# chalharu/rust-compression

Hardware: AMD Instinct MI355X
Metric: BZip2 level-9 encode MB/s (input bytes, HBM-resident in and out: the kernels' rate; value_end_to_end is host buffer to host buffer at the C ABI) (higher is better)
Workload: dtype u8/u32

## Files before the change

rust-compression_amd/csrc/k_huff.hip:

```cpp
#include "bzgpu.h"
#include <cstdlib>

namespace bzgpu {

constexpr u32 kHuffThreads = 512;

__device__ __forceinline__ u32 weight_add(u32 x, u32 y)
{
    const u32 dx = x & 0xFFu, dy = y & 0xFFu;
    return ((x & 0xFFFFFF00u) + (y & 0xFFFFFF00u)) | (1u + (dx > dy ? dx : dy));
}

__device__ void down_heap(u32 *buf, u32 nn, u32 len)
{
    const u32 tmp = buf[nn];
    u32 leaf = (nn << 1) + 1;
    while (leaf < len) {
        if (leaf + 1 < len && buf[buf[leaf]] > buf[buf[leaf + 1]]) leaf += 1;
        if (buf[tmp] < buf[buf[leaf]]) break;
        buf[nn] = buf[leaf];
        nn = leaf;
        leaf = (nn << 1) + 1;
    }
    buf[nn] = tmp;
// ... 966 lines not shown
                    nacc -= 32u;
                }
            }
        }
        if (nacc) atomicOr(&s_buf[widx], (u32)(acc >> 32));
    }
    __syncthreads();
    for (u32 q = tid * 4u; q < nwords; q += kEmitThreads * 4u) {
        const u32 w = base + q;
        if (w > wf && w + 3u < wl && w + 3u < kStreamWords) {
            *reinterpret_cast<uint4 *>(stream + w) = *reinterpret_cast<const uint4 *>(s_buf + q);
            continue;
        }
#pragma unroll
        for (u32 j = 0; j < 4; ++j) {
            const u32 ww = w + j;
            if (ww < wf || ww > wl || ww >= kStreamWords) continue;
            const u32 v = s_buf[q + j];
            if (ww != wf && ww != wl) stream[ww] = v;
            else if (v) atomicOr(&stream[ww], v);
        }
    }
}

constexpr u32 kSweepThreads = 256;
constexpr u32 kSweepTilesX = 11;
constexpr u32 kTabArena = 6 * (3 * kMaxAlpha + 4);

__device__ __forceinline__ u32 huff_group_num(u32 mtf_count)
{
    if (mtf_count < 200) return 2;
    if (mtf_count < 600) return 3;
    if (mtf_count < 1200) return 4;
    if (mtf_count < 2400) return 5;
    return 6;
}

__device__ __forceinline__ void lm_wave_sync()
{
    __builtin_amdgcn_fence(__ATOMIC_ACQ_REL, "workgroup");
    __builtin_amdgcn_wave_barrier();
}
__device__ void lm_code_lengths_wave(const u32 *rfreq, u32 n, u32 *scr, u32 scr_words, u32 row, u8 *out, u32 lane)
{
    const u32 lim = kLim;
    u32 *map = scr;
    u32 *sfreq = map + kMaxAlpha;
    u32 *c = sfreq + kMaxAlpha;
    u32 *misc = c + kMaxAlpha;
    u32 *max_elem = misc, *b = misc + 20, *cur = misc + 40;
    u32 *val = misc + 64 + kMaxAlpha;
    u32 *ty = val + lim * row;
    u32 *w = scr + scr_words - kMaxAlpha;
    for (u32 i = lane; i < n; i += 64u) {
        const u32 f = rfreq[i];
        w[i] = (f > 1u ? f : 1u) << 8;
    }
    lm_wave_sync();
    for (u32 i = lane; i < n; i += 64u) {
        const u32 f = w[i];
        u32 r = 0;
        for (u32 q = 0; q < n; ++q) {
            const u32 x = w[q];
            r += (x > f || (x == f && q < i)) ? 1u : 0u;
        }
        sfreq[r] = f;
        map[r] = i;
    }
    if (lane == 0) {
        for (u32 j = 0; j < lim; ++j) { max_elem[j] = 0; b[j] = 0; cur[j] = 0; }
        u32 excess = (1u << lim) - n;
        const u32 half = 1u << (lim - 1);
        max_elem[lim - 1] = n;
        for (u32 j = 0; j < lim; ++j) {
            if (excess >= half) {
                b[j] = 1;
                excess -= half;
            }
            excess <<= 1;
            if (lim >= 2 + j) max_elem[lim - 2 - j] = max_elem[lim - 1 - j] / 2 + n;
        }
        max_elem[0] = b[0];
        for (u32 j = 1; j < lim; ++j)
            if (max_elem[j] > 2 * max_elem[j - 1] + b[j]) max_elem[j] = 2 * max_elem[j - 1] + b[j];
    }
    lm_wave_sync();
    for (u32 j = 0; j < lim; ++j)
        for (u32 t = lane; t < max_elem[j]; t += 64u) { val[j * row + t] = 0; ty[j * row + t] = 0; }
    for (u32 i = lane; i < n; i += 64u) c[i] = lim;
    lm_wave_sync();
    for (u32 t = lane; t < n && t < max_elem[lim - 1]; t += 64u) {
        val[(lim - 1) * row + t] = sfreq[t];
        ty[(lim - 1) * row + t] = t;
    }
    if (lane == 0 && b[lim - 1] == 1) {
        c[0] -= 1;
        cur[lim - 1] += 1;
    }
    lm_wave_sync();
    const u32 last_leaf = sfreq[n - 1];
    for (u32 j = lim - 1; j > 0;) {
        const u32 next0 = cur[j], me = max_elem[j], cap = max_elem[j - 1];
        const u32 K = (me > next0 + 1u) ? (me - next0) / 2u : 0u;
        u32 *vj = val + j * row, *dv = val + (j - 1) * row, *dt = ty + (j - 1) * row;
        for (u32 k0 = 0; k0 < K; k0 += 64u) {
            const u32 k = k0 + lane;
            u32 pk = 0;
            if (k < K) pk = weight_add(vj[next0 + 2u * k], vj[next0 + 2u * k + 1u]);
            lm_wave_sync();
            if (k < K) vj[k] = pk;
        }
        lm_wave_sync();
        for (u32 k = lane; k < K; k += 64u) {
            const u32 pk = vj[k];
            if (pk > last_leaf) {
                u32 lo = 0, hi = n;
                while (lo < hi) {
                    const u32 mid = (lo + hi) >> 1;
                    if (sfreq[mid] >= pk) lo = mid + 1u;
                    else hi = mid;
                }
                const u32 pos = k + lo;
                if (pos < cap) {
                    dv[pos] = pk;
                    dt[pos] = n;
                }
            }
        }
        for (u32 i = lane; i < n; i += 64u) {
            const u32 sf = sfreq[i];
            u32 lo = 0, hi = K;
            while (lo < hi) {
                const u32 mid = (lo + hi) >> 1;
                if (vj[mid] > sf) lo = mid + 1u;
                else hi = mid;
            }
            const u32 pos = i + lo;
            if (pos < cap) {
                dv[pos] = sf;
                dt[pos] = i;
            }
        }
        lm_wave_sync();
        j -= 1;
        if (lane == 0) cur[j] = 0;
        lm_wave_sync();
        if (b[j] == 1) {
            u32 need = 1;
            for (u32 li = j; need > 0u && li < lim; ++li) {
                const u32 c0 = cur[li];
                u32 npk = 0;
                for (u32 t0 = 0; t0 < need; t0 += 64u) {
                    const u32 t = t0 + lane;
                    bool isp = false;
                    if (t < need) {
                        const u32 x = ty[li * row + c0 + t];
                        if (x == n) isp = true;
                        else c[x] -= 1;
                    }
                    npk += (u32)__popcll(__ballot(isp));
                }
                lm_wave_sync();
                if (lane == 0) cur[li] = c0 + need;
                need = 2u * npk;
                lm_wave_sync();
            }
        }
        lm_wave_sync();
    }
    for (u32 i = lane; i < n; i += 64u) out[map[i]] = (u8)c[i];
    lm_wave_sync();
}

template <u32 THREADS>
__device__ __forceinline__ void stage_symbols_n(u32 *s_sym, const u16 *__restrict__ mtf, u32 g0, u32 mtf_count)
{
    const u32 first = g0 * kGSize;
    const u32 avail = mtf_count - first;
    const u32 want = THREADS * kGSize;
    const u32 nsym = avail < want ? avail : want;
    const u32 ndw = (nsym + 1u) >> 1;
    const u32 *src = reinterpret_cast<const u32 *>(mtf + first);
    u32 v[kGSize / 2];
#pragma unroll
    for (u32 k = 0; k < kGSize / 2; ++k) {
        const u32 i = threadIdx.x + k * THREADS;
        v[k] = (i < ndw) ? src[i] : 0u;
    }
#pragma unroll
    for (u32 k = 0; k < kGSize / 2; ++k) {
        const u32 i = threadIdx.x + k * THREADS;
        if (i < ndw) s_sym[i] = v[k];
    }
}

constexpr u32 kTabPipeBlocks = 320;
template <u32 kTabThreads>
__global__ __launch_bounds__(kTabThreads) void k_huff_tables(HuffArgs a, u32 iter)
{
    __shared__ u8 s_len[6][kMaxAlpha + 6];
    __shared__ u32 s_rfreq[6][kMaxAlpha];
    __shared__ __attribute__((aligned(16))) u32 s_arena[kTabArena];
    __shared__ u32 s_need[6];
    __shared__ u32 s_lmcount;
    static_assert(kTabArena >= 6 * (3 * kMaxAlpha + 4) && (3 * kMaxAlpha + 4) % 2 == 0, "the heap work arrays fit the arena, 8-byte aligned");
    const u32 lb = blockIdx.x, tid = threadIdx.x, lane = threadIdx.x & 63u, wv = threadIdx.x >> 6;
    const BlockOut &bo = a.out[lb];
    const u32 mtf_count = bo.mtf_count;
    const u32 alpha = bo.in_use_count + 2;
    const u32 group_num = huff_group_num(mtf_count);
    const u32 *mtf_freq = a.mtf_freq + (size_t)lb * kMaxAlpha;
    u32 *rfreq = a.rfreq + (size_t)lb * 6 * kMaxAlpha;
    u8 *glen = a.glen + (size_t)lb * 6 * (kMaxAlpha + 6);
    const bool tab_lane = tid < group_num;
    const u32 tb = tid;
    if (tid == 0) s_lmcount = 0;
    if (iter == 0) {
        if (tid == 0) {
            u32 rem = mtf_count;
            int gs = 0;
            for (u32 k = 0; k < group_num; ++k) {
                const u32 n_part = group_num - k;
                const u32 t_freq = rem / n_part;
                int ge = gs - 1;
                u32 a_freq = 0;
                while (a_freq < t_freq && ge < (int)alpha - 1) {
                    ge += 1;
                    a_freq += mtf_freq[ge];
                }
                if (ge > gs && n_part != group_num && n_part != 1 && (((group_num - n_part) & 1u) == 1u)) {
                    a_freq -= mtf_freq[ge];
                    ge -= 1;
                }
                s_need[group_num - 1 - k] = (u32)gs | ((u32)(ge + 1) << 16);
                rem -= a_freq;
                gs = ge + 1;
            }
            a.hlm[lb] = 0;
        }
        for (u32 i = tid; i < 6 * kMaxAlpha; i += kTabThreads) rfreq[i] = 0;
        __syncthreads();
        for (u32 i = tid; i < group_num * alpha; i += kTabThreads) {
            const u32 t = i / alpha, sym = i - t * alpha, rg = s_need[t];
            s_len[t][sym] = (sym >= (rg & 0xFFFFu) && sym < (rg >> 16)) ? 0 : 15;
        }
        __syncthreads();
    } else {
        for (u32 i = tid; i < 6 * kMaxAlpha; i += kTabThreads) {
            (&s_rfreq[0][0])[i] = rfreq[i];
            rfreq[i] = 0;
        }
        __syncthreads();
        if constexpr (kTabThreads >= 384) {
            const bool on = wv < group_num;
            const u32 gq = on ? wv : 0u;
            const int lm = heap_code_lengths_pipe(s_rfreq[gq], alpha, s_arena + gq * (3 * kMaxAlpha + 4), s_len[gq], lane, on);
            if (on && lane == 0) s_need[wv] = (u32)lm;
        } else {
            if (tab_lane) s_need[tb] = (u32)heap_code_lengths_w(s_rfreq[tb], alpha, s_arena + tb * (3 * kMaxAlpha + 4), s_len[tb]);
        }
        __syncthreads();
        const u32 row = 2u * alpha + 4u;
        const u32 need = 5u * kMaxAlpha + 64u + 2u * kLim * row;
        const u32 slots = kTabArena / need;
        u32 my_rank = 0, any = 0;
        for (u32 t = 0; t < group_num; ++t) {
            if (t < tb) my_rank += s_need[t] ? 1u : 0u;
            any += s_need[t] ? 1u : 0u;
        }
        (void)my_rank;
        if (any) {
            if (slots) {
                if (wv == 0) {
                    for (u32 t = 0; t < group_num; ++t) {
                        if (s_need[t]) {
                            lm_code_lengths_wave(s_rfreq[t], alpha, s_arena, need, row, s_len[t], lane);
                            if (lane == 0) s_lmcount += 1;
                        }
                    }
                }
                __syncthreads();
            } else {
                for (u32 t = wv; t < group_num; t += kTabThreads / 64u) {
                    if (s_need[t]) {
                        lm_code_lengths_wave(s_rfreq[t], alpha, a.lm_scratch + ((size_t)lb * 6 + t) * kLmWords, kLmWords, kLmRow,
                                             s_len[t], lane);
                        if (lane == 0) atomicAdd(&s_lmcount, 1u);
                    }
                }
                __syncthreads();
            }
        }
    }
    for (u32 i = tid; i < 6 * (kMaxAlpha + 6); i += kTabThreads) glen[i] = (&s_len[0][0])[i];
    unsigned long long *pack = a.pack + (size_t)lb * kMaxAlpha;
    for (u32 i = tid; i < alpha; i += kTabThreads) {
        unsigned long long p = 0;
        for (u32 t = 0; t < group_num; ++t) p |= (unsigned long long)s_len[t][i] << (10 * t);
        pack[i] = p;
    }
    if (tid == 0 && s_lmcount) a.hlm[lb] += s_lmcount;
}

__global__ __launch_bounds__(kSweepThreads) void k_huff_sweep(HuffArgs a, u32 iter)
{
    __shared__ unsigned long long s_pack[kMaxAlpha];
    __shared__ u32 s_pass[8];
    __shared__ u32 s_rfreq[6][kMaxAlpha];
    __shared__ u32 s_sym[kSweepThreads * kGSize / 2];
    const u32 lb = blockIdx.y, tid = threadIdx.x;
    const u32 mtf_count = a.out[lb].mtf_count;
    const u32 n_selectors = (mtf_count + kGSize - 1) / kGSize;
    if (blockIdx.x * kSweepThreads >= n_selectors) return;
    const u32 alpha = a.out[lb].in_use_count + 2;
    const u32 group_num = huff_group_num(mtf_count);
    const u16 *mtf = a.mtf + (size_t)lb * a.mtf_stride;
    u8 *selector = a.selector + (size_t)lb * kSelStride;
    const unsigned long long *pack = a.pack + (size_t)lb * kMaxAlpha;
    for (u32 i = tid; i < alpha; i += kSweepThreads) s_pack[i] = pack[i];
    for (u32 i = tid; i < 6 * kMaxAlpha; i += kSweepThreads) (&s_rfreq[0][0])[i] = 0;
    if (tid < 8) s_pass[tid] = 0;
    for (u32 g0 = blockIdx.x * kSweepThreads; g0 < n_selectors; g0 += kSweepTilesX * kSweepThreads) {
        __syncthreads();
        stage_symbols_n<kSweepThreads>(s_sym, mtf, g0, mtf_count);
        __syncthreads();
        const u32 g = g0 + tid;
        u32 bt_mine = 0xFFFFFFFFu, bc_mine = 0;
        if (g < n_selectors) {
            const u32 gs = g * kGSize;
            const u32 cnt = (gs + kGSize < mtf_count) ? kGSize : mtf_count - gs;
            const u32 *my = s_sym + tid * (kGSize / 2);
            unsigned long long cost = 0, c8 = 0;
            u32 big = 0;
            if (cnt == kGSize) {
#pragma unroll 5
                for (u32 k = 0; k < kGSize / 2; ++k) {
                    const u32 dw = my[k];
                    const u32 s0 = dw & 0xFFFFu, s1 = dw >> 16;
                    cost += s_pack[s0];
                    cost += s_pack[s1];
                    if (s0 < 8u) c8 += 1ull << (8u * s0);
                    else ++big;
                    if (s1 < 8u) c8 += 1ull << (8u * s1);
                    else ++big;
                }
            } else {
                for (u32 i = 0; i < cnt; ++i) {
                    const u32 sy = (my[i >> 1] >> ((i & 1u) * 16u)) & 0xFFFFu;
                    cost += s_pack[sy];
                    if (sy < 8u) c8 += 1ull << (8u * sy);
                    else ++big;
                }
            }
            u32 bt = 0, bc = (u32)(cost & 1023u);
            for (u32 t = 1; t < group_num; ++t) {
                const u32 ct = (u32)((cost >> (10 * t)) & 1023u);
                if (ct < bc) {
                    bc = ct;
                    bt = t;
                }
            }
            selector[g] = (u8)bt;
            bt_mine = bt;
            bc_mine = bc;
            if (big) {
                for (u32 i = 0; i < cnt; ++i) {
                    const u32 sy = (my[i >> 1] >> ((i & 1u) * 16u)) & 0xFFFFu;
                    if (sy >= 8u) atomicAdd(&s_rfreq[bt][sy], 1u);
                }
            }
#pragma unroll
            for (u32 q = 0; q < 8; ++q) {
                const u32 c = (u32)(c8 >> (8u * q)) & 0xFFu;
                if (c) atomicAdd(&s_rfreq[bt][q], c);
            }
        }
        if (a.pass_stats) {
            const u32 wtot = wave_sum(bc_mine);
            u32 mine = 0;
#pragma unroll
            for (u32 t = 0; t < 6; ++t) {
                const u32 c = (u32)__popcll(__ballot(bt_mine == t));
                mine = (tid & 63u) == t + 1u ? c : mine;
            }
            if ((tid & 63u) == 0u) mine = wtot;
            if ((tid & 63u) < 7u && mine) atomicAdd(&s_pass[tid & 63u], mine);
        }
    }
    __syncthreads();
    u32 *rfreq = a.rfreq + (size_t)lb * 6 * kMaxAlpha;
    for (u32 i = tid; i < group_num * kMaxAlpha; i += kSweepThreads) {
        const u32 c = (&s_rfreq[0][0])[i];
        if (c) atomicAdd(&rfreq[i], c);
    }
    if (a.pass_stats && tid < 7 && s_pass[tid]) atomicAdd(&a.pass_stats[((size_t)lb * 4 + iter) * 8 + tid], s_pass[tid]);
}

__global__ __launch_bounds__(kSweepThreads) void k_huff_gbits(HuffArgs a)
{
    __shared__ u8 s_len[6][kMaxAlpha + 6];
    __shared__ u32 s_sym[kSweepThreads * kGSize / 2];
    const u32 lb = blockIdx.y, tid = threadIdx.x;
    const u32 mtf_count = a.out[lb].mtf_count;
    const u32 n_selectors = (mtf_count + kGSize - 1) / kGSize;
    if (blockIdx.x * kSweepThreads >= n_selectors) return;
    const u16 *mtf = a.mtf + (size_t)lb * a.mtf_stride;
    const u8 *selector = a.selector + (size_t)lb * kSelStride;
    const u8 *glen = a.glen + (size_t)lb * 6 * (kMaxAlpha + 6);
    u32 *gbo = a.group_bitoff + (size_t)lb * kGboStride;
    for (u32 i = tid; i < 6 * (kMaxAlpha + 6); i += kSweepThreads) (&s_len[0][0])[i] = glen[i];
    for (u32 g0 = blockIdx.x * kSweepThreads; g0 < n_selectors; g0 += kSweepTilesX * kSweepThreads) {
        __syncthreads();
        stage_symbols_n<kSweepThreads>(s_sym, mtf, g0, mtf_count);
        __syncthreads();
        const u32 g = g0 + tid;
        if (g < n_selectors) {
            const u32 gs = g * kGSize;
            const u32 cnt = (gs + kGSize < mtf_count) ? kGSize : mtf_count - gs;
            const u32 *my = s_sym + tid * (kGSize / 2);
            const u8 *l = s_len[selector[g]];
            u32 bits = 0;
            if (cnt == kGSize) {
#pragma unroll 5
                for (u32 k = 0; k < kGSize / 2; ++k) {
                    const u32 d = my[k];
                    bits += (u32)l[d & 0xFFFFu] + (u32)l[d >> 16];
                }
            } else {
                for (u32 i = 0; i < cnt; ++i) bits += l[(my[i >> 1] >> ((i & 1u) * 16u)) & 0xFFFFu];
            }
            gbo[g] = bits;
        }
    }
}

__global__ __launch_bounds__(kHuffThreads) void k_huff_header(HuffArgs a)
{
    __shared__ u8 s_len[6][kMaxAlpha + 6];
    __shared__ u32 s_scan[kHuffThreads / 64];
    __shared__ u32 s_run;
    __shared__ u32 s_first[6][24], s_lcount[6][24];
    const u32 lb = blockIdx.x;
    const u32 tid = threadIdx.x, lane = tid & 63u, wave = tid >> 6;
    BlockOut &bo = a.out[lb];
    const u32 mtf_count = bo.mtf_count;
    const u32 alpha = bo.in_use_count + 2;
    const u32 group_num = huff_group_num(mtf_count);
    const u32 n_selectors = (mtf_count + kGSize - 1) / kGSize;
    const u8 *selector = a.selector + (size_t)lb * kSelStride;
    const u8 *glen = a.glen + (size_t)lb * 6 * (kMaxAlpha + 6);
    const bool tab_lane = (wave == 0 && lane < group_num);
    const u32 tb = lane;
    for (u32 i = tid; i < 6 * (kMaxAlpha + 6); i += kHuffThreads) (&s_len[0][0])[i] = glen[i];
    if (tid < 6 * 24) (&s_lcount[0][0])[tid] = 0;
    __syncthreads();
    for (u32 i = tid; i < group_num * alpha; i += kHuffThreads) {
        const u32 t = i / alpha, sy = i - t * alpha;
        atomicAdd(&s_lcount[t][s_len[t][sy]], 1u);
    }
    __syncthreads();
    if (tid < group_num) {
        u32 code = 0;
        for (u32 l = 1; l < 24; ++l) {
            code = (code + s_lcount[tid][l - 1]) << 1;
            s_first[tid][l] = code;
        }
    }
    __syncthreads();
    u32 *code_len = a.code_len + (size_t)lb * 6 * kMaxAlpha;
    u32 my_max = 0;
    for (u32 i = tid; i < group_num * alpha; i += kHuffThreads) {
        const u32 t = i / alpha, sy = i - t * alpha;
        const u32 l = s_len[t][sy];
        u32 r = 0;
        for (u32 q = 0; q < sy; ++q) r += (s_len[t][q] == l) ? 1u : 0u;
        code_len[t * kMaxAlpha + sy] = (s_first[t][l] + r) | (l << 24);
        my_max = l > my_max ? l : my_max;
    }
#pragma unroll
    for (u32 dd = 32; dd >= 1; dd >>= 1) {
        const u32 o = __shfl_xor(my_max, dd, 64);
        my_max = o > my_max ? o : my_max;
    }
    if (tid == 0) s_run = 0;
    if (tid < kHuffThreads / 64) s_scan[tid] = 0;
    __syncthreads();
    if (lane == 0) atomicMax(&s_scan[0], my_max);
    __syncthreads();
    const u32 max_len = s_scan[0];
    __syncthreads();

    u32 *gbo = a.group_bitoff + (size_t)lb * kGboStride;
    for (u32 g0 = 0; g0 < n_selectors; g0 += kHuffThreads) {
        const u32 g = g0 + tid;
        const u32 bits = (g < n_selectors) ? gbo[g] : 0u;
        const u32 inc = wave_incl_sum(bits);
        if (lane == 63) s_scan[wave] = inc;
        __syncthreads();
        u32 carry = s_run, tot = 0;
        for (u32 k = 0; k < kHuffThreads / 64; ++k) {
            if (k < wave) carry += s_scan[k];
            tot += s_scan[k];
        }
        if (g < n_selectors) gbo[g] = carry + inc - bits;
        __syncthreads();
        if (tid == 0) s_run += tot;
        __syncthreads();
    }
    const u32 payload_bits = s_run;

    u32 *stream = a.stream + (size_t)lb * kStreamWords;
    const u32 *ubits = a.inuse_bits + lb * 8;
    u32 in_use16 = 0, used_ranges = 0;
    for (u32 i = 0; i < 16; ++i) {
        const u32 half = (ubits[i >> 1] >> ((i & 1u) * 16u)) & 0xFFFFu;
        in_use16 = (in_use16 << 1) | (half ? 1u : 0u);
        used_ranges += half ? 1u : 0u;
    }
    const u32 sel_bit0 = 48u + 32u + 1u + 24u + 16u + 16u * used_ranges + 3u + 15u;
    const u32 seg = (n_selectors + kHuffThreads - 1) / kHuffThreads;
    const u32 g_lo = tid * seg < n_selectors ? tid * seg : n_selectors;
    const u32 g_hi = (g_lo + seg < n_selectors) ? g_lo + seg : n_selectors;
    int last[6];
#pragma unroll
    for (int t = 0; t < 6; ++t) last[t] = -1000000;
    for (u32 g = g_lo; g < g_hi; ++g) {
        const u32 v = selector[g];
#pragma unroll
        for (int t = 0; t < 6; ++t)
            if ((u32)t == v) last[t] = (int)g;
    }
    int start_last[6];
#pragma unroll
    for (int t = 0; t < 6; ++t) {
        const int inc = wave_incl_max32(last[t]);
        if (lane == 63) s_scan[wave] = (u32)inc;
        __syncthreads();
        int carry = -1000000;
        for (u32 k = 0; k < wave; ++k) carry = (int)s_scan[k] > carry ? (int)s_scan[k] : carry;
        const int prev = __shfl_up(inc, 1, 64);
        int ex = (lane == 0) ? -1000000 : prev;
        ex = ex > carry ? ex : carry;
        start_last[t] = (ex < 0) ? -(t + 1) : ex;
        __syncthreads();
    }
    u32 my_bits = 0;
    {
        int cur[6];
#pragma unroll
        for (int t = 0; t < 6; ++t) cur[t] = start_last[t];
        for (u32 g = g_lo; g < g_hi; ++g) {
            const u32 v = selector[g];
            int lv = 0;
#pragma unroll
            for (int t = 0; t < 6; ++t)
                if ((u32)t == v) lv = cur[t];
            u32 pos = 0;
#pragma unroll
            for (int t = 0; t < 6; ++t) pos += (cur[t] > lv) ? 1u : 0u;
#pragma unroll
            for (int t = 0; t < 6; ++t)
                if ((u32)t == v) cur[t] = (int)g;
            my_bits += pos + 1u;
        }
    }
    u32 sel_off, sel_total;
    {
        const u32 inc = wave_incl_sum(my_bits);
        if (lane == 63) s_scan[wave] = inc;
        __syncthreads();
        u32 carry = 0, tot = 0;
        for (u32 k = 0; k < kHuffThreads / 64; ++k) {
            if (k < wave) carry += s_scan[k];
            tot += s_scan[k];
        }
        sel_off = carry + inc - my_bits;
        sel_total = tot;
        __syncthreads();
    }
    const u32 tab_bit0 = sel_bit0 + sel_total;
    if (tab_lane) {
        const u8 *l = s_len[tb];
        u32 nb = 5, curr = l[0];
        for (u32 i = 0; i < alpha; ++i) {
            const u32 li = l[i];
            nb += 2u * (li > curr ? li - curr : curr - li) + 1u;
            curr = li;
        }
        s_first[tb][0] = nb;
    }
    __syncthreads();
    u32 tab_off[7];
    tab_off[0] = tab_bit0;
    for (u32 t = 0; t < 6; ++t) tab_off[t + 1] = tab_off[t] + (t < group_num ? s_first[t][0] : 0u);
    const u32 hb = tab_off[group_num];
    for (u32 w = tid; w <= (hb >> 5); w += kHuffThreads) stream[w] = 0;
    __syncthreads();
    auto put = [&](u32 bitpos, u32 v, u32 nbits) {
        const u32 w = bitpos >> 5, o = bitpos & 31u;
        const unsigned long long x = (unsigned long long)v << (64u - o - nbits);
        atomicOr(&stream[w], (u32)(x >> 32));
        if ((u32)x) atomicOr(&stream[w + 1], (u32)x);
    };
    if (tid == 0) {
        put(0, 0x314159u, 24);
        put(24, 0x265359u, 24);
        put(48, a.crc[lb], 32);
        put(81, a.orig_ptr[lb], 24);
        put(105, in_use16, 16);
        u32 bp = 121;
        for (u32 i = 0; i < 16; ++i) {
            const u32 half = (ubits[i >> 1] >> ((i & 1u) * 16u)) & 0xFFFFu;
            if (half) {
                put(bp, __brev(half) >> 16, 16);
                bp += 16;
            }
        }
        put(bp, group_num, 3);
        put(bp + 3, n_selectors, 15);
    }
    {
        int cur[6];
#pragma unroll
        for (int t = 0; t < 6; ++t) cur[t] = start_last[t];
        u32 bp = sel_bit0 + sel_off;
        for (u32 g = g_lo; g < g_hi; ++g) {
            const u32 v = selector[g];
            int lv = 0;
#pragma unroll
            for (int t = 0; t < 6; ++t)
                if ((u32)t == v) lv = cur[t];
            u32 pos = 0;
#pragma unroll
            for (int t = 0; t < 6; ++t) pos += (cur[t] > lv) ? 1u : 0u;
#pragma unroll
            for (int t = 0; t < 6; ++t)
                if ((u32)t == v) cur[t] = (int)g;
            put(bp, (1u << (pos + 1u)) - 2u, pos + 1u);
            bp += pos + 1u;
        }
    }
    if (tab_lane) {
        const u8 *l = s_len[tb];
        u32 bp = tab_off[tb];
        u32 curr = l[0];
        put(bp, curr, 5);
        bp += 5;
        for (u32 i = 0; i < alpha; ++i) {
            const u32 li = l[i];
            while (curr < li) { put(bp, 2, 2); bp += 2; curr += 1; }
            while (curr > li) { put(bp, 3, 2); bp += 2; curr -= 1; }
            bp += 1;
        }
    }
    if (tid == 0) {
        bo.header_bits = hb;
        bo.pad = used_ranges | (sel_total << 5);
        bo.total_bits = (u64)hb + payload_bits;
        bo.group_num = group_num;
        bo.n_selectors = n_selectors;
        bo.max_len = max_len;
        bo.lm_tables = a.hlm[lb];
        bo.crc = a.crc[lb];
        bo.orig_ptr = a.orig_ptr[lb];
        if ((u64)hb + payload_bits + 96u > (u64)kStreamWords * 32u) atomicExch(a.error_flag, 1u);
    }
    {
        const u64 tbits = (u64)hb + payload_bits;
        u32 w0 = (hb >> 5) + 1u;
        u32 w1 = (u32)(tbits >> 5) + 2u;
        if (w1 > kStreamWords) w1 = kStreamWords;
        for (u32 w = w0 + tid; w < w1; w += kHuffThreads) stream[w] = 0;
    }
}

void launch_huffman(hipStream_t st, const HuffArgs &a)
{
    static const bool split = !(getenv("BZ_HUFF_SPLIT") && atoi(getenv("BZ_HUFF_SPLIT")) == 0);
    if (a.pass_stats) (void)hipMemsetAsync(a.pass_stats, 0, (size_t)a.nb * 32 * sizeof(u32), st);
    if (split) {
        const dim3 sweep_grid(kSweepTilesX, a.nb);
        const bool pipe = a.nb <= kTabPipeBlocks;
        auto tables = [&](u32 iter) {
            if (pipe) hipLaunchKernelGGL(k_huff_tables<384>, dim3(a.nb), dim3(384), 0, st, a, iter);
            else hipLaunchKernelGGL(k_huff_tables<64>, dim3(a.nb), dim3(64), 0, st, a, iter);
        };
        tables(0u);
        for (u32 iter = 1; iter <= 4; ++iter) {
            hipLaunchKernelGGL(k_huff_sweep, sweep_grid, dim3(kSweepThreads), 0, st, a, iter - 1u);
            tables(iter);
        }
        hipLaunchKernelGGL(k_huff_gbits, sweep_grid, dim3(kSweepThreads), 0, st, a);
        hipLaunchKernelGGL(k_huff_header, dim3(a.nb), dim3(kHuffThreads), 0, st, a);
    } else {
        hipLaunchKernelGGL(k_huffman, dim3(a.nb), dim3(kHuffThreads), 0, st, a);
    }
    hipLaunchKernelGGL(k_emit_payload, dim3((kMaxSelectors + 255) / 256, a.nb), dim3(256), 0, st, a);
}

__global__ void k_probe_code_lengths(const u32 *freq, u32 alpha, u8 *out, u32 *lm_scr, int *lm_flag)
{
    __shared__ u32 s_buf[2 * kMaxAlpha + 4];
    __shared__ __attribute__((aligned(16))) u32 s_arena_w[3 * kMaxAlpha + 4];
    __shared__ u32 s_f[kMaxAlpha];
    __shared__ u8 s_o[kMaxAlpha + 6], s_o2[kMaxAlpha + 6], s_o3[kMaxAlpha + 6];
    __shared__ int s_lm, s_bad;
    if (threadIdx.x == 0) {
        for (u32 i = 0; i < alpha; ++i) s_f[i] = freq[i];
        const int lm = heap_code_lengths(s_f, alpha, s_buf, s_o);
        {
            const int lm2 = heap_code_lengths_w(s_f, alpha, s_arena_w, s_o2);
            s_bad = lm2 != lm ? 1 : 0;
            for (u32 i = 0; i < alpha; ++i)
                if (s_o2[i] != s_o[i]) s_bad = 1;
        }
        if (lm) lm_code_lengths(s_f, alpha, lm_scr, kLmWords, kLmRow, s_o);
        *lm_flag = lm;
        s_lm = lm;
    }
    __syncthreads();
    {
        const int lm3 = heap_code_lengths_pipe(s_f, alpha, s_arena_w, s_o3, threadIdx.x, true);
        __syncthreads();
        if (threadIdx.x == 0) {
            if (lm3 != s_lm) s_bad = 1;
            for (u32 i = 0; i < alpha; ++i)
                if (s_o3[i] != s_o2[i]) s_bad = 1;
        }
        __syncthreads();
    }
    if (s_lm) {
        lm_code_lengths_wave(s_f, alpha, lm_scr, kLmWords, kLmRow, s_o2, threadIdx.x);
        __syncthreads();
        if (threadIdx.x == 0)
            for (u32 i = 0; i < alpha; ++i)
                if (s_o2[i] != s_o[i]) s_o[i] = 0xFF;
    }
    __syncthreads();
    if (threadIdx.x == 0)
        for (u32 i = 0; i < alpha; ++i) out[i] = s_bad ? (u8)0xFE : s_o[i];
}

void launch_probe_code_lengths(hipStream_t st, const u32 *d_freq, u32 alpha, u8 *d_out, u32 *lm_scr,
                               int *d_flag)
{
    hipLaunchKernelGGL(k_probe_code_lengths, dim3(1), dim3(64), 0, st, d_freq, alpha, d_out, lm_scr, d_flag);
}

}
```

Baseline: 15390.

## Interleave hot-symbol counts into sweep cost table and wave-reduce frequency updates

The sweep kernel gets a WAVE variant, on by default. It stores each symbol's packed cost next to a one-hot count word for symbols below 8, so a single 128-bit LDS load gives both cost and hot-symbol counts. Symbols of 8 or more are recorded in a bitmask and walked with ffs, removing the separate rescan of the group. Per-group hot-symbol counts are reduced across the wave with DPP before one atomic per lane, which cuts LDS atomic contention. This doubles the s_pack shared footprint, adds a per-group loop of DPP reductions, and includes optional cycle-counter instrumentation behind a macro.

```diff
diff --git a/rust-compression_amd/csrc/k_huff.hip b/rust-compression_amd/csrc/k_huff.hip
--- a/rust-compression_amd/csrc/k_huff.hip
+++ b/rust-compression_amd/csrc/k_huff.hip
@@ -1292,9 +1292,32 @@
     if (tid == 0 && s_lmcount) a.hlm[lb] += s_lmcount;
 }
 
+#ifdef BZ_SWEEP_TIMING
+__device__ u32 g_sweep_marks[8];
+#define SW_T(k) do { __syncthreads(); const u64 t_ = __builtin_readcyclecounter(); if (threadIdx.x == 0) atomicAdd(&g_sweep_marks[k], (u32)((t_ - t_prev) >> 4)); t_prev = t_; } while (0)
+#else
+#define SW_T(k) do { } while (0)
+#endif
+
+__device__ __forceinline__ u32 wave_sum_dpp(u32 v)
+{
+    v += (u32)__builtin_amdgcn_update_dpp(0, (int)v, 0xB1 , 0xf, 0xf, false);
+    v += (u32)__builtin_amdgcn_update_dpp(0, (int)v, 0x4E , 0xf, 0xf, false);
+    v += (u32)__builtin_amdgcn_update_dpp(0, (int)v, 0x141 , 0xf, 0xf, false);
+    v += (u32)__builtin_amdgcn_update_dpp(0, (int)v, 0x140 , 0xf, 0xf, false);
+    v += (u32)__builtin_amdgcn_update_dpp(0, (int)v, 0x142 , 0xa, 0xf, false);
+    v += (u32)__builtin_amdgcn_update_dpp(0, (int)v, 0x143 , 0xc, 0xf, false);
+    return (u32)__builtin_amdgcn_readlane((int)v, 63);
+}
+
+template <bool WAVE>
 __global__ __launch_bounds__(kSweepThreads) void k_huff_sweep(HuffArgs a, u32 iter)
 {
-    __shared__ unsigned long long s_pack[kMaxAlpha];
+#ifdef BZ_SWEEP_TIMING
+    u64 t_prev = __builtin_readcyclecounter();
+#endif
+    typedef unsigned long long u64x2 __attribute__((ext_vector_type(2)));
+    __shared__ __attribute__((aligned(16))) unsigned long long s_pack[WAVE ? 2 * kMaxAlpha : kMaxAlpha];
     __shared__ u32 s_pass[8];
     __shared__ u32 s_rfreq[6][kMaxAlpha];
     __shared__ u32 s_sym[kSweepThreads * kGSize / 2];
@@ -1307,41 +1330,67 @@
     const u16 *mtf = a.mtf + (size_t)lb * a.mtf_stride;
     u8 *selector = a.selector + (size_t)lb * kSelStride;
     const unsigned long long *pack = a.pack + (size_t)lb * kMaxAlpha;
-    for (u32 i = tid; i < alpha; i += kSweepThreads) s_pack[i] = pack[i];
+    for (u32 i = tid; i < alpha; i += kSweepThreads) {
+        if constexpr (WAVE) {
+            s_pack[2 * i] = pack[i];
+            s_pack[2 * i + 1] = i < 8u ? 1ull << (8u * i) : 0ull;
+        } else {
+            s_pack[i] = pack[i];
+        }
+    }
     for (u32 i = tid; i < 6 * kMaxAlpha; i += kSweepThreads) (&s_rfreq[0][0])[i] = 0;
     if (tid < 8) s_pass[tid] = 0;
+    SW_T(0);
     for (u32 g0 = blockIdx.x * kSweepThreads; g0 < n_selectors; g0 += kSweepTilesX * kSweepThreads) {
         __syncthreads();
         stage_symbols_n<kSweepThreads>(s_sym, mtf, g0, mtf_count);
         __syncthreads();
+        SW_T(1);
         const u32 g = g0 + tid;
+        const bool live = g < n_selectors;
+        const u32 gs = g * kGSize;
+        const u32 cnt = !live ? 0u : (gs + kGSize < mtf_count) ? kGSize : mtf_count - gs;
+        const u32 *my = s_sym + tid * (kGSize / 2);
         u32 bt_mine = 0xFFFFFFFFu, bc_mine = 0;
-        if (g < n_selectors) {
-            const u32 gs = g * kGSize;
-            const u32 cnt = (gs + kGSize < mtf_count) ? kGSize : mtf_count - gs;
-            const u32 *my = s_sym + tid * (kGSize / 2);
-            unsigned long long cost = 0, c8 = 0;
-            u32 big = 0;
-            if (cnt == kGSize) {
+        unsigned long long cost = 0, c8 = 0, at = 0;
+        u32 big = 0;
+        if (cnt == kGSize) {
 #pragma unroll 5
-                for (u32 k = 0; k < kGSize / 2; ++k) {
-                    const u32 dw = my[k];
-                    const u32 s0 = dw & 0xFFFFu, s1 = dw >> 16;
+            for (u32 k = 0; k < kGSize / 2; ++k) {
+                const u32 dw = my[k];
+                const u32 s0 = dw & 0xFFFFu, s1 = dw >> 16;
+                if constexpr (WAVE) {
+                    const u64x2 e0 = reinterpret_cast<const u64x2 *>(s_pack)[s0], e1 = reinterpret_cast<const u64x2 *>(s_pack)[s1];
+                    cost += e0.x;
+                    cost += e1.x;
+                    c8 += e0.y;
+                    c8 += e1.y;
+                } else {
                     cost += s_pack[s0];
                     cost += s_pack[s1];
+                }
+                if constexpr (WAVE) {
+                    const u32 w = dw + 0x01F801F8u;
+                    const u32 in = ((w >> 9) & 1u) | ((w >> 24) & 2u);
+                    at = (at >> 2) | ((unsigned long long)in << (kGSize - 2));
+                } else {
                     if (s0 < 8u) c8 += 1ull << (8u * s0);
                     else ++big;
                     if (s1 < 8u) c8 += 1ull << (8u * s1);
                     else ++big;
                 }
-            } else {
-                for (u32 i = 0; i < cnt; ++i) {
-                    const u32 sy = (my[i >> 1] >> ((i & 1u) * 16u)) & 0xFFFFu;
-                    cost += s_pack[sy];
-                    if (sy < 8u) c8 += 1ull << (8u * sy);
-                    else ++big;
-                }
-            }
+            }
+        } else {
+            for (u32 i = 0; i < cnt; ++i) {
+                const u32 sy = (my[i >> 1] >> ((i & 1u) * 16u)) & 0xFFFFu;
+                cost += s_pack[WAVE ? 2u * sy : sy];
+                if (sy < 8u) c8 += 1ull << (8u * sy);
+                else if constexpr (WAVE) at |= 1ull << i;
+                else ++big;
+            }
+        }
+        SW_T(2);
+        if (live) {
             u32 bt = 0, bc = (u32)(cost & 1023u);
             for (u32 t = 1; t < group_num; ++t) {
                 const u32 ct = (u32)((cost >> (10 * t)) & 1023u);
@@ -1353,17 +1402,46 @@
             selector[g] = (u8)bt;
             bt_mine = bt;
             bc_mine = bc;
+        }
+        SW_T(3);
+        if constexpr (WAVE) {
+            while (at) {
+                const u32 i = (u32)__ffsll((long long)at) - 1u;
+                at &= at - 1ull;
+                const u32 sy = (my[i >> 1] >> ((i & 1u) * 16u)) & 0xFFFFu;
+                atomicAdd(&s_rfreq[bt_mine][sy], 1u);
+            }
+            SW_T(4);
+            const u32 lo = (u32)c8, hi = (u32)(c8 >> 32);
+            const u32 w0 = (lo & 0xFFu) | ((lo & 0xFF00u) << 8), w1 = ((lo >> 16) & 0xFFu) | ((lo >> 8) & 0xFF0000u);
+            const u32 w2 = (hi & 0xFFu) | ((hi & 0xFF00u) << 8), w3 = ((hi >> 16) & 0xFFu) | ((hi >> 8) & 0xFF0000u);
+            const u32 lane = tid & 63u;
+            for (u32 t = 0; t < group_num; ++t) {
+                const bool in = bt_mine == t;
+                if (!__ballot(in)) continue;
+                const u32 x0 = wave_sum_dpp(in ? w0 : 0u), x1 = wave_sum_dpp(in ? w1 : 0u);
+                const u32 x2 = wave_sum_dpp(in ? w2 : 0u), x3 = wave_sum_dpp(in ? w3 : 0u);
+                const u32 pr = (lane & 4u) ? ((lane & 2u) ? x3 : x2) : ((lane & 2u) ? x1 : x0);
+                const u32 c = (pr >> ((lane & 1u) * 16u)) & 0xFFFFu;
+                if (lane < 8u && c) atomicAdd(&s_rfreq[t][lane], c);
+            }
+            SW_T(5);
+        } else {
             if (big) {
                 for (u32 i = 0; i < cnt; ++i) {
                     const u32 sy = (my[i >> 1] >> ((i & 1u) * 16u)) & 0xFFFFu;
-                    if (sy >= 8u) atomicAdd(&s_rfreq[bt][sy], 1u);
-                }
-            }
-#pragma unroll
-            for (u32 q = 0; q < 8; ++q) {
-                const u32 c = (u32)(c8 >> (8u * q)) & 0xFFu;
-                if (c) atomicAdd(&s_rfreq[bt][q], c);
-            }
+                    if (sy >= 8u) atomicAdd(&s_rfreq[bt_mine][sy], 1u);
+                }
+            }
+            SW_T(4);
+            if (live) {
+#pragma unroll
+                for (u32 q = 0; q < 8; ++q) {
+                    const u32 c = (u32)(c8 >> (8u * q)) & 0xFFu;
+                    if (c) atomicAdd(&s_rfreq[bt_mine][q], c);
+                }
+            }
+            SW_T(5);
         }
         if (a.pass_stats) {
             const u32 wtot = wave_sum(bc_mine);
@@ -1376,6 +1454,7 @@
             if ((tid & 63u) == 0u) mine = wtot;
             if ((tid & 63u) < 7u && mine) atomicAdd(&s_pass[tid & 63u], mine);
         }
+        SW_T(6);
     }
     __syncthreads();
     u32 *rfreq = a.rfreq + (size_t)lb * 6 * kMaxAlpha;
@@ -1384,6 +1463,7 @@
         if (c) atomicAdd(&rfreq[i], c);
     }
     if (a.pass_stats && tid < 7 && s_pass[tid]) atomicAdd(&a.pass_stats[((size_t)lb * 4 + iter) * 8 + tid], s_pass[tid]);
+    SW_T(7);
 }
 
 __global__ __launch_bounds__(kSweepThreads) void k_huff_gbits(HuffArgs a)
@@ -1667,6 +1747,7 @@
 void launch_huffman(hipStream_t st, const HuffArgs &a)
 {
     static const bool split = !(getenv("BZ_HUFF_SPLIT") && atoi(getenv("BZ_HUFF_SPLIT")) == 0);
+    static const bool wave_form = !(getenv("BZ_SWEEP_FORM") && atoi(getenv("BZ_SWEEP_FORM")) == 0);
     if (a.pass_stats) (void)hipMemsetAsync(a.pass_stats, 0, (size_t)a.nb * 32 * sizeof(u32), st);
     if (split) {
         const dim3 sweep_grid(kSweepTilesX, a.nb);
@@ -1677,9 +1758,21 @@
         };
         tables(0u);
         for (u32 iter = 1; iter <= 4; ++iter) {
-            hipLaunchKernelGGL(k_huff_sweep, sweep_grid, dim3(kSweepThreads), 0, st, a, iter - 1u);
+            if (wave_form) hipLaunchKernelGGL(k_huff_sweep<true>, sweep_grid, dim3(kSweepThreads), 0, st, a, iter - 1u);
+            else hipLaunchKernelGGL(k_huff_sweep<false>, sweep_grid, dim3(kSweepThreads), 0, st, a, iter - 1u);
             tables(iter);
         }
+#ifdef BZ_SWEEP_TIMING
+        {
+            (void)hipStreamSynchronize(st);
+            u32 rt[8] = {};
+            (void)hipMemcpyFromSymbol(rt, HIP_SYMBOL(g_sweep_marks), sizeof(rt));
+            fprintf(stderr, "  k_huff_sweep<%d> cycles/16 per phase (set-up, staging, cost loop, argmin + selector, walk of symbols >= 8, "
+                            "hot counts, figures, flush): %u %u %u %u %u %u %u %u\n", (int)wave_form, rt[0], rt[1], rt[2], rt[3], rt[4], rt[5], rt[6], rt[7]);
+            const u32 zero[8] = {};
+            (void)hipMemcpyToSymbol(HIP_SYMBOL(g_sweep_marks), zero, sizeof(zero));
+        }
+#endif
         hipLaunchKernelGGL(k_huff_gbits, sweep_grid, dim3(kSweepThreads), 0, st, a);
         hipLaunchKernelGGL(k_huff_header, dim3(a.nb), dim3(kHuffThreads), 0, st, a);
     } else {
```

Measured after the change: 15370. No clear change (-0.1%).
